# hiimmuc/SpeakerVerification

Hardware: AMD Instinct MI355X
Metric: embeddings/sec (2 s @16 kHz) (higher is better)
Workload: dtype bf16

## Files before the change

speakerverification_amd/csrc/asp_x3.hip:

```cpp
#include "common.h"
#include "kernels.h"

namespace svhip {

namespace {

typedef __attribute__((address_space(3))) void lds_void;
typedef __attribute__((address_space(1))) const void gbl_void;

constexpr int AX_THREADS = 512;
constexpr int AX_PLANE = 32 * 256;
constexpr int AX_RAW = 32 * 512;
constexpr int AX_XSLAB = 32 * 128;
constexpr int AX_NSLOT = 3;
constexpr int AX_XRING = 2 * AX_PLANE + 2 * AX_RAW;
constexpr int AX_LDS = AX_XRING + 8 * AX_NSLOT * AX_XSLAB;
constexpr float AX_L2E = 1.4426950408889634f;

__global__ __launch_bounds__(AX_THREADS, 2) void asp_x3_kernel(AspX3Params p) {
    extern __shared__ __attribute__((aligned(16))) char smem[];
    char* planes = smem;
    char* raw = smem + 2 * AX_PLANE;
    const int ncg = p.C >> 8;
    int b, cg;
    {
        const int id = blockIdx.x, full = (p.B >> 3) * 8 * ncg;
        if (id < full) {
            const int slot = id >> 3;
            b = (slot / ncg) * 8 + (id & 7);
            cg = slot - (slot / ncg) * ncg;
        } else {
            const int q = id - full;
            b = (p.B >> 3) * 8 + q / ncg;
            cg = q - (q / ncg) * ncg;
        }
    }
    const int tid = threadIdx.x, lane = tid & 63;
    const int wave = __builtin_amdgcn_readfirstlane(tid >> 6);
    char* xring = smem + AX_XRING + wave * AX_NSLOT * AX_XSLAB;
    const int r = lane & 31, h = lane >> 5;
    const int cw = cg * 256 + wave * 32;
    const int c = cw + r;
    const int T = p.T;
    const int nt = (T + 31) >> 5;

    bf16x8 wh[8], wl[8];
    {
        const char* wrow = reinterpret_cast<const char*>(p.Ws32) + (int64_t)c * 512;
#pragma unroll
        for (int ks = 0; ks < 8; ++ks) {
            const char* q = wrow + (ks >> 1) * 128 + ((ks & 1) * 16 + 8 * h) * 2;
            wh[ks] = *reinterpret_cast<const bf16x8*>(q);
            wl[ks] = *reinterpret_cast<const bf16x8*>(q + 64);
        }
    }
    const float mref = p.mref[(int64_t)b * p.mref_ld + c];
    const char* abase = reinterpret_cast<const char*>(p.att + (int64_t)b * T * 128) + (lane & 31) * 16;
    const char* xbase = reinterpret_cast<const char*>(p.X + (int64_t)b * T * p.ldx + cw) + (lane & 7) * 16;
    const int64_t xrow = (int64_t)p.ldx * 4;
    auto dma_att = [&](int mt, int buf) {
#pragma unroll
        for (int i = 0; i < 2; ++i) {
            const int f = min(mt * 32 + 4 * wave + 2 * i + (lane >> 5), T - 1);
            __builtin_amdgcn_global_load_lds((gbl_void*)(abase + (int64_t)f * 512), (lds_void*)(raw + buf * AX_RAW + (4 * wave + 2 * i) * 512), 16, 0, CPOL_NT);
        }
    };
    auto dma_x = [&](int mt, int slot) {
#pragma unroll
        for (int i = 0; i < 4; ++i) {
            const int f = min(mt * 32 + 8 * i + (lane >> 3), T - 1);
            __builtin_amdgcn_global_load_lds((gbl_void*)(xbase + f * xrow), (lds_void*)(xring + slot * AX_XSLAB + i * 1024), 16, 0, CPOL_NT);
        }
    };
    const int sfr = tid >> 4;
    const int soff = sfr * 256 + (((tid & 15) ^ (sfr & 15)) << 4);
    auto convert = [&](int buf) {
        const f32x4* q = reinterpret_cast<const f32x4*>(raw + buf * AX_RAW + sfr * 512 + (tid & 15) * 32);
        const f32x4 v0 = q[0], v1 = q[1];
        x3x8_t hi, lo;
#pragma unroll
        for (int j = 0; j < 8; ++j) {
            const float v = j < 4 ? v0[j] : v1[j - 4];
            const x3_t hb = x3_hi(v);
            hi[j] = hb;
            lo[j] = x3_lo(v, hb);
        }
        *reinterpret_cast<x3x8_t*>(planes + soff) = hi;
        *reinterpret_cast<x3x8_t*>(planes + AX_PLANE + soff) = lo;
    };

    auto lds_barrier = [&]() {
        asm volatile("s_waitcnt lgkmcnt(0)" ::: "memory");
        __builtin_amdgcn_s_barrier();
        asm volatile("" ::: "memory");
    };
    float m = -INFINITY, se = 0.0f, s1 = 0.0f, s2 = 0.0f;
    dma_att(0, 0);
    dma_x(0, 0);
    dma_att(1, 1);
    dma_x(1, 1);
    asm volatile("s_waitcnt vmcnt(10)" ::: "memory");
    lds_barrier();
    convert(0);
    lds_barrier();
    int slot = 0;
    for (int mt = 0; mt < nt; ++mt) {
        const int fill = slot == 0 ? 2 : slot - 1;
        dma_att(mt + 2, mt & 1);
        dma_x(mt + 2, fill);
        f32x16 acc;
#pragma unroll
        for (int e = 0; e < 16; ++e) acc[e] = 0.0f;
#pragma unroll
        for (int ks = 0; ks < 8; ++ks) {
            const int o = r * 256 + (((2 * ks + h) ^ (r & 15)) << 4);
            const bf16x8 ah = *reinterpret_cast<const bf16x8*>(planes + o);
            const bf16x8 al = *reinterpret_cast<const bf16x8*>(planes + AX_PLANE + o);
            acc = X3H::mfma32(al, wh[ks], acc);
            acc = X3H::mfma32(ah, wl[ks], acc);
            acc = X3H::mfma32(ah, wh[ks], acc);
        }
        if (mt * 32 + 32 > T) {
#pragma unroll
            for (int e = 0; e < 16; ++e) {
                const int f = mt * 32 + (e & 3) + 8 * (e >> 2) + 4 * h;
                acc[e] = f < T ? acc[e] : -INFINITY;
            }
        }
        float tmax = fmaxf(acc[0], acc[1]);
#pragma unroll
        for (int e = 2; e < 16; e += 2) tmax = fmaxf(fmaxf(acc[e], acc[e + 1]), tmax);
        const float mnew = fmaxf(m, tmax);
        const float mm = mnew == -INFINITY ? 0.0f : mnew;
        const float fs = __builtin_amdgcn_exp2f((m - mm) * AX_L2E);
        se *= fs; s1 *= fs; s2 *= fs;
        const float mb = mm * AX_L2E;
        asm volatile("s_waitcnt vmcnt(12)" ::: "memory");
        const float* xs = reinterpret_cast<const float*>(xring + slot * AX_XSLAB) + r;
#pragma unroll
        for (int e = 0; e < 16; ++e) {
            const float w = __builtin_amdgcn_exp2f(fmaf(acc[e], AX_L2E, -mb));
            const float d = xs[((e & 3) + 8 * (e >> 2) + 4 * h) * 32] - mref;
            const float wd = w * d;
            se += w;
            s1 += wd;
            s2 = fmaf(wd, d, s2);
        }
        m = mnew;
        slot = slot == 2 ? 0 : slot + 1;
        asm volatile("s_waitcnt vmcnt(10)" ::: "memory");
        lds_barrier();
        convert((mt + 1) & 1);
        lds_barrier();
    }
    asm volatile("s_waitcnt vmcnt(0)" ::: "memory");
    const float mo = __shfl_xor(m, 32), seo = __shfl_xor(se, 32), s1o = __shfl_xor(s1, 32), s2o = __shfl_xor(s2, 32);
    const float M = fmaxf(m, mo);
    const float MM = M == -INFINITY ? 0.0f : M;
    const float f1 = __builtin_amdgcn_exp2f((m - MM) * AX_L2E), f2 = __builtin_amdgcn_exp2f((mo - MM) * AX_L2E);
    const float SE = se * f1 + seo * f2, S1 = s1 * f1 + s1o * f2, S2 = s2 * f1 + s2o * f2;
    if (h == 0) {
        const float md = S1 / SE;
        const float mean = mref + md;
        const float sd = sqrtf(fmaxf(S2 / SE - md * md, p.eps));
        const int C = p.C;
        if (p.pooled_raw) {
            p.pooled_raw[(int64_t)b * 2 * C + c] = mean;
            p.pooled_raw[(int64_t)b * 2 * C + C + c] = sd;
        }
        p.pooled_bn[(int64_t)b * 2 * C + c] = fmaf(mean, p.bn_scale[c], p.bn_shift[c]);
        p.pooled_bn[(int64_t)b * 2 * C + C + c] = fmaf(sd, p.bn_scale[C + c], p.bn_shift[C + c]);
    }
}

constexpr int AB_ATT = 32 * 256;
constexpr int AB_XSLAB = 32 * 64;
constexpr int AB_LDS = 2 * AB_ATT + 8 * AX_NSLOT * AB_XSLAB;

__global__ __launch_bounds__(AX_THREADS, 4) void asp_bf16_kernel(AspFusedParams p, const float* __restrict__ mref_all, int mref_ld, int Bn) {
    extern __shared__ __attribute__((aligned(16))) char smem[];
    const int ncg = p.C >> 8;
    int b, cg;
    {
        const int id = blockIdx.x, full = (Bn >> 3) * 8 * ncg;
        if (id < full) {
            const int slot = id >> 3;
            b = (slot / ncg) * 8 + (id & 7);
            cg = slot - (slot / ncg) * ncg;
        } else {
            const int q = id - full;
            b = (Bn >> 3) * 8 + q / ncg;
            cg = q - (q / ncg) * ncg;
        }
    }
    const int tid = threadIdx.x, lane = tid & 63;
    const int wave = __builtin_amdgcn_readfirstlane(tid >> 6);
    char* xring = smem + 2 * AB_ATT + wave * AX_NSLOT * AB_XSLAB;
    const int r = lane & 31, h = lane >> 5;
    const int cw = cg * 256 + wave * 32;
    const int c = cw + r;
    const int T = p.T;
    const int nt = (T + 31) >> 5;

    bf16x8 wf[8];
    {
        const char* wrow = reinterpret_cast<const char*>(p.W) + ((int64_t)c * p.Kp + 8 * h) * 2;
#pragma unroll
        for (int ks = 0; ks < 8; ++ks) wf[ks] = *reinterpret_cast<const bf16x8*>(wrow + ks * 32);
    }
    const float mref = mref_all[(int64_t)b * mref_ld + c];
    const int sfr = tid >> 4;
    const char* abase = reinterpret_cast<const char*>(p.att) + (int64_t)b * T * 256 + (((tid & 15) ^ (sfr & 15)) << 4);
    const char* xbase = reinterpret_cast<const char*>(p.X) + ((int64_t)b * T * p.ldx + cw) * 2 + (lane & 3) * 16;
    const int64_t xrow = (int64_t)p.ldx * 2;
    auto dma_att = [&](int mt, int buf) {
        const int f = min(mt * 32 + sfr, T - 1);
        __builtin_amdgcn_global_load_lds((gbl_void*)(abase + (int64_t)f * 256), (lds_void*)(smem + buf * AB_ATT + wave * 1024), 16, 0, 0);
    };
    auto dma_x = [&](int mt, int slot) {
#pragma unroll
        for (int i = 0; i < 2; ++i) {
            const int f = min(mt * 32 + 16 * i + (lane >> 2), T - 1);
            __builtin_amdgcn_global_load_lds((gbl_void*)(xbase + f * xrow), (lds_void*)(xring + slot * AB_XSLAB + i * 1024), 16, 0, 0);
        }
    };
    auto lds_barrier = [&]() {
        asm volatile("s_waitcnt lgkmcnt(0)" ::: "memory");
        __builtin_amdgcn_s_barrier();
        asm volatile("" ::: "memory");
    };
    float m = -INFINITY, se = 0.0f, s1 = 0.0f, s2 = 0.0f;
    dma_x(0, 0);
    dma_att(0, 0);
    dma_x(1, 1);
    asm volatile("s_waitcnt vmcnt(2)" ::: "memory");
    lds_barrier();
    int slot = 0;
    for (int mt = 0; mt < nt; ++mt) {
        const int buf = mt & 1;
        const int fill = slot == 0 ? 2 : slot - 1;
        dma_att(mt + 1, buf ^ 1);
        dma_x(mt + 2, fill);
        f32x16 acc;
#pragma unroll
        for (int e = 0; e < 16; ++e) acc[e] = 0.0f;
        const char* at = smem + buf * AB_ATT + r * 256;
#pragma unroll
        for (int ks = 0; ks < 8; ++ks) {
            const bf16x8 a = *reinterpret_cast<const bf16x8*>(at + (((2 * ks + h) ^ (r & 15)) << 4));
            acc = __builtin_amdgcn_mfma_f32_32x32x16_bf16(a, wf[ks], acc, 0, 0, 0);
        }
        if (mt * 32 + 32 > T) {
#pragma unroll
            for (int e = 0; e < 16; ++e) {
                const int f = mt * 32 + (e & 3) + 8 * (e >> 2) + 4 * h;
                acc[e] = f < T ? acc[e] : -INFINITY;
            }
        }
        float tmax = fmaxf(acc[0], acc[1]);
#pragma unroll
        for (int e = 2; e < 16; e += 2) tmax = fmaxf(fmaxf(acc[e], acc[e + 1]), tmax);
        const float mnew = fmaxf(m, tmax);
        const float mm = mnew == -INFINITY ? 0.0f : mnew;
        const float fs = __builtin_amdgcn_exp2f((m - mm) * AX_L2E);
        se *= fs; s1 *= fs; s2 *= fs;
        const float mb = mm * AX_L2E;
        const uint16_t* xs = reinterpret_cast<const uint16_t*>(xring + slot * AB_XSLAB) + r;
#pragma unroll
        for (int e = 0; e < 16; ++e) {
            const float w = __builtin_amdgcn_exp2f(fmaf(acc[e], AX_L2E, -mb));
            const float xv = __uint_as_float((uint32_t)xs[((e & 3) + 8 * (e >> 2) + 4 * h) * 32] << 16);
            const float d = xv - mref;
            const float wd = w * d;
            se += w;
            s1 += wd;
            s2 = fmaf(wd, d, s2);
        }
        m = mnew;
        slot = slot == 2 ? 0 : slot + 1;
        asm volatile("s_waitcnt vmcnt(2)" ::: "memory");
        lds_barrier();
    }
    asm volatile("s_waitcnt vmcnt(0)" ::: "memory");
    const float mo = __shfl_xor(m, 32), seo = __shfl_xor(se, 32), s1o = __shfl_xor(s1, 32), s2o = __shfl_xor(s2, 32);
    const float M = fmaxf(m, mo);
    const float MM = M == -INFINITY ? 0.0f : M;
    const float f1 = __builtin_amdgcn_exp2f((m - MM) * AX_L2E), f2 = __builtin_amdgcn_exp2f((mo - MM) * AX_L2E);
    const float SE = se * f1 + seo * f2, S1 = s1 * f1 + s1o * f2, S2 = s2 * f1 + s2o * f2;
    if (h == 0) {
        const float md = S1 / SE;
        const float mean = mref + md;
        const float sd = sqrtf(fmaxf(S2 / SE - md * md, p.eps));
        const int C = p.C;
        if (p.pooled_raw) {
            p.pooled_raw[(int64_t)b * 2 * C + c] = mean;
            p.pooled_raw[(int64_t)b * 2 * C + C + c] = sd;
        }
        p.pooled_bn[(int64_t)b * 2 * C + c] = fmaf(mean, p.bn_scale[c], p.bn_shift[c]);
        p.pooled_bn[(int64_t)b * 2 * C + C + c] = fmaf(sd, p.bn_scale[C + c], p.bn_shift[C + c]);
    }
}

}

hipError_t launch_asp_bf16(const AspFusedParams& p, const float* mref, int mref_ld, int B, hipStream_t stream) {
    if (p.T < 1 || p.C % 256 != 0 || p.Kp != 128 || !p.att || !p.W || !p.X || !mref || !p.pooled_bn || B <= 0 || p.ldx % 8 != 0) return hipErrorInvalidValue;
    static DeviceOnce once;
    hipError_t e = set_max_dynamic_lds(once, reinterpret_cast<const void*>(asp_bf16_kernel), AB_LDS);
    if (e != hipSuccess) return e;
    hipLaunchKernelGGL(asp_bf16_kernel, dim3((p.C / 256) * B), dim3(AX_THREADS), AB_LDS, stream, p, mref, mref_ld, B);
    return hipGetLastError();
}

bool asp_x3_supported(int T, int C, int att_channels, int K) {
    return T >= 1 && C % 256 == 0 && att_channels == 128 && K == 128;
}

hipError_t launch_asp_x3(const AspX3Params& p, int B, hipStream_t stream) {
    if (!asp_x3_supported(p.T, p.C, 128, 128) || !p.att || !p.Ws32 || !p.X || !p.mref || !p.pooled_bn || B <= 0) return hipErrorInvalidValue;
    if (((reinterpret_cast<uintptr_t>(p.att) | reinterpret_cast<uintptr_t>(p.Ws32)) & 15) != 0) return hipErrorInvalidValue;
    static DeviceOnce once;
    hipError_t e = set_max_dynamic_lds(once, reinterpret_cast<const void*>(asp_x3_kernel), AX_LDS);
    if (e != hipSuccess) return e;
    AspX3Params q = p;
    q.B = B;
    hipLaunchKernelGGL(asp_x3_kernel, dim3((p.C / 256) * B), dim3(AX_THREADS), AX_LDS, stream, q);
    return hipGetLastError();
}

}
```

Measured before the change: 57890.

## Software-pipeline ASP bf16 kernel: overlap next tile MFMA with current softmax stats

```diff
diff --git a/speakerverification_amd/csrc/asp_x3.hip b/speakerverification_amd/csrc/asp_x3.hip
--- a/speakerverification_amd/csrc/asp_x3.hip
+++ b/speakerverification_amd/csrc/asp_x3.hip
@@ -7,6 +7,7 @@
 
 typedef __attribute__((address_space(3))) void lds_void;
 typedef __attribute__((address_space(1))) const void gbl_void;
+typedef __attribute__((address_space(3))) const bf16x8 lds_frag;
 
 constexpr int AX_THREADS = 512;
 constexpr int AX_PLANE = 32 * 256;
@@ -176,6 +177,12 @@
 constexpr int AB_ATT = 32 * 256;
 constexpr int AB_XSLAB = 32 * 64;
 constexpr int AB_LDS = 2 * AB_ATT + 8 * AX_NSLOT * AB_XSLAB;
+constexpr int AB_AHEAD = 2;
+#define AB_XREAD(j, e) asm volatile("ds_read_u16_d16_hi %0, %1 offset:%2" : "+v"(xr[j]) : "v"(xa), "n"(((e) & 3) * 64 + ((e) >> 2) * 512) : "memory")
+#define AB_XREREAD(j, e, used) asm volatile("ds_read_u16_d16_hi %0, %1 offset:%2" : "+v"(xr[j]) : "v"(xa), "n"(((e) & 3) * 64 + ((e) >> 2) * 512), "v"(used) : "memory")
+#define AB_XREADS() do { AB_XREAD(0, 0); AB_XREAD(1, 1); AB_XREAD(2, 2); AB_XREAD(3, 3); AB_XREAD(4, 4); AB_XREAD(5, 5); AB_XREAD(6, 6); AB_XREAD(7, 7); } while (0)
+#define AB_XWAIT() do { asm volatile("s_waitcnt lgkmcnt(0)" ::: "memory"); \
+    asm volatile("" : "+v"(xr[0]), "+v"(xr[1]), "+v"(xr[2]), "+v"(xr[3]), "+v"(xr[4]), "+v"(xr[5]), "+v"(xr[6]), "+v"(xr[7]) :: "memory"); } while (0)
 
 __global__ __launch_bounds__(AX_THREADS, 4) void asp_bf16_kernel(AspFusedParams p, const float* __restrict__ mref_all, int mref_ld, int Bn) {
     extern __shared__ __attribute__((aligned(16))) char smem[];
@@ -210,18 +217,18 @@
     }
     const float mref = mref_all[(int64_t)b * mref_ld + c];
     const int sfr = tid >> 4;
-    const char* abase = reinterpret_cast<const char*>(p.att) + (int64_t)b * T * 256 + (((tid & 15) ^ (sfr & 15)) << 4);
-    const char* xbase = reinterpret_cast<const char*>(p.X) + ((int64_t)b * T * p.ldx + cw) * 2 + (lane & 3) * 16;
-    const int64_t xrow = (int64_t)p.ldx * 2;
+    const char* abase = reinterpret_cast<const char*>(p.att) + (int64_t)b * T * 256;
+    const char* xbase = reinterpret_cast<const char*>(p.X) + ((int64_t)b * T * p.ldx + cw) * 2;
+    const uint32_t aoff = ((tid & 15) ^ (sfr & 15)) << 4, xoff = (lane & 3) * 16, xrow = (uint32_t)p.ldx * 2;
     auto dma_att = [&](int mt, int buf) {
         const int f = min(mt * 32 + sfr, T - 1);
-        __builtin_amdgcn_global_load_lds((gbl_void*)(abase + (int64_t)f * 256), (lds_void*)(smem + buf * AB_ATT + wave * 1024), 16, 0, 0);
+        __builtin_amdgcn_global_load_lds((gbl_void*)(abase + (aoff + (uint32_t)f * 256)), (lds_void*)(smem + buf * AB_ATT + wave * 1024), 16, 0, 0);
     };
     auto dma_x = [&](int mt, int slot) {
 #pragma unroll
         for (int i = 0; i < 2; ++i) {
             const int f = min(mt * 32 + 16 * i + (lane >> 2), T - 1);
-            __builtin_amdgcn_global_load_lds((gbl_void*)(xbase + f * xrow), (lds_void*)(xring + slot * AB_XSLAB + i * 1024), 16, 0, 0);
+            __builtin_amdgcn_global_load_lds((gbl_void*)(xbase + (xoff + (uint32_t)f * xrow)), (lds_void*)(xring + slot * AB_XSLAB + i * 1024), 16, 0, 0);
         }
     };
     auto lds_barrier = [&]() {
@@ -230,56 +237,90 @@
         asm volatile("" ::: "memory");
     };
     float m = -INFINITY, se = 0.0f, s1 = 0.0f, s2 = 0.0f;
-    dma_x(0, 0);
-    dma_att(0, 0);
-    dma_x(1, 1);
-    asm volatile("s_waitcnt vmcnt(2)" ::: "memory");
-    lds_barrier();
-    int slot = 0;
-    for (int mt = 0; mt < nt; ++mt) {
-        const int buf = mt & 1;
-        const int fill = slot == 0 ? 2 : slot - 1;
-        dma_att(mt + 1, buf ^ 1);
-        dma_x(mt + 2, fill);
-        f32x16 acc;
-#pragma unroll
-        for (int e = 0; e < 16; ++e) acc[e] = 0.0f;
-        const char* at = smem + buf * AB_ATT + r * 256;
-#pragma unroll
-        for (int ks = 0; ks < 8; ++ks) {
-            const bf16x8 a = *reinterpret_cast<const bf16x8*>(at + (((2 * ks + h) ^ (r & 15)) << 4));
-            acc = __builtin_amdgcn_mfma_f32_32x32x16_bf16(a, wf[ks], acc, 0, 0, 0);
-        }
-        if (mt * 32 + 32 > T) {
-#pragma unroll
-            for (int e = 0; e < 16; ++e) {
-                const int f = mt * 32 + (e & 3) + 8 * (e >> 2) + 4 * h;
-                acc[e] = f < T ? acc[e] : -INFINITY;
+    float xr[8];
+#pragma unroll
+    for (int e = 0; e < 8; ++e) xr[e] = 0.0f;
+    const uint32_t xa0 = (uint32_t)(uintptr_t)(lds_void*)xring + r * 2 + h * 256;
+    int slot = 2;
+    auto pre = [&](int t) {
+        asm volatile("s_waitcnt vmcnt(2)" ::: "memory");
+        lds_barrier();
+        dma_att(t + 2, t & 1);
+        dma_x(t + 2, slot == 0 ? 2 : slot - 1);
+    };
+    auto step = [&](f32x16& as, f32x16& am, const int t, auto SM, auto MM) {
+        constexpr bool sm = decltype(SM)::value, mmf = decltype(MM)::value;
+        const uint32_t at = (uint32_t)(uintptr_t)(lds_void*)smem + ((t + 1) & 1) * AB_ATT + r * 256 + ((h ^ (r & 15)) << 4);
+        auto frag = [&](int ks) { return *(lds_frag*)(uintptr_t)(at ^ (ks << 5)); };
+        bf16x8 af[8];
+        float mnew = m, mb = 0.0f;
+        const uint32_t xa = xa0 + slot * AB_XSLAB;
+        if constexpr (sm) {
+            AB_XREADS();
+            if (t * 32 + 32 > T) {
+#pragma unroll
+                for (int e = 0; e < 16; ++e) {
+                    const int f = t * 32 + (e & 3) + 8 * (e >> 2) + 4 * h;
+                    as[e] = f < T ? as[e] : -INFINITY;
+                }
             }
-        }
-        float tmax = fmaxf(acc[0], acc[1]);
-#pragma unroll
-        for (int e = 2; e < 16; e += 2) tmax = fmaxf(fmaxf(acc[e], acc[e + 1]), tmax);
-        const float mnew = fmaxf(m, tmax);
-        const float mm = mnew == -INFINITY ? 0.0f : mnew;
-        const float fs = __builtin_amdgcn_exp2f((m - mm) * AX_L2E);
-        se *= fs; s1 *= fs; s2 *= fs;
-        const float mb = mm * AX_L2E;
-        const uint16_t* xs = reinterpret_cast<const uint16_t*>(xring + slot * AB_XSLAB) + r;
+            float tmax = fmaxf(as[0], as[1]);
+#pragma unroll
+            for (int e = 2; e < 16; e += 2) tmax = fmaxf(fmaxf(as[e], as[e + 1]), tmax);
+            mnew = fmaxf(m, tmax);
+            const float mm = mnew == -INFINITY ? 0.0f : mnew;
+            const float fs = __builtin_amdgcn_exp2f((m - mm) * AX_L2E);
+            se *= fs; s1 *= fs; s2 *= fs;
+            mb = mm * AX_L2E;
+        }
+        if constexpr (mmf) {
+#pragma unroll
+            for (int e = 0; e < 16; ++e) am[e] = 0.0f;
+#pragma unroll
+            for (int ks = 0; ks < AB_AHEAD; ++ks) af[ks] = frag(ks);
+        }
 #pragma unroll
         for (int e = 0; e < 16; ++e) {
-            const float w = __builtin_amdgcn_exp2f(fmaf(acc[e], AX_L2E, -mb));
-            const float xv = __uint_as_float((uint32_t)xs[((e & 3) + 8 * (e >> 2) + 4 * h) * 32] << 16);
-            const float d = xv - mref;
-            const float wd = w * d;
-            se += w;
-            s1 += wd;
-            s2 = fmaf(wd, d, s2);
+            if ((e & 1) == 0) __builtin_amdgcn_sched_barrier(0);
+            if constexpr (mmf) {
+                if ((e & 1) == 0) {
+                    const int ks = e >> 1;
+                    if (ks + AB_AHEAD < 8) af[ks + AB_AHEAD] = frag(ks + AB_AHEAD);
+                    am = __builtin_amdgcn_mfma_f32_32x32x16_bf16(af[ks], wf[ks], am, 0, 0, 0);
+                }
+            }
+            if constexpr (sm) {
+                if ((e & 7) == 0) AB_XWAIT();
+                const float d = xr[e & 7] - mref;
+                if (e < 8) AB_XREREAD(e, e + 8, d);
+                const float w = __builtin_amdgcn_exp2f(fmaf(as[e], AX_L2E, -mb));
+                const float wd = w * d;
+                se += w;
+                s1 += wd;
+                s2 = fmaf(wd, d, s2);
+            }
         }
         m = mnew;
         slot = slot == 2 ? 0 : slot + 1;
-        asm volatile("s_waitcnt vmcnt(2)" ::: "memory");
-        lds_barrier();
+    };
+    const std::true_type yes;
+    const std::false_type no;
+    f32x16 acc0, acc1;
+    dma_att(0, 0);
+    dma_x(0, 0);
+    pre(-1);
+    step(acc1, acc0, -1, no, yes);
+    int t = 0;
+    for (; t + 1 < nt; t += 2) {
+        pre(t);
+        step(acc0, acc1, t, yes, yes);
+        pre(t + 1);
+        if (t + 2 < nt) step(acc1, acc0, t + 1, yes, yes);
+        else step(acc1, acc0, t + 1, yes, no);
+    }
+    if (t < nt) {
+        pre(t);
+        step(acc0, acc1, t, yes, no);
     }
     asm volatile("s_waitcnt vmcnt(0)" ::: "memory");
     const float mo = __shfl_xor(m, 32), seo = __shfl_xor(se, 32), s1o = __shfl_xor(s1, 32), s2o = __shfl_xor(s2, 32);
@@ -292,6 +333,9 @@
         const float mean = mref + md;
         const float sd = sqrtf(fmaxf(S2 / SE - md * md, p.eps));
         const int C = p.C;
+        int rr = threadIdx.x & 31;
+        asm volatile("" : "+v"(rr));
+        const int c = cw + rr;
         if (p.pooled_raw) {
             p.pooled_raw[(int64_t)b * 2 * C + c] = mean;
             p.pooled_raw[(int64_t)b * 2 * C + C + c] = sd;
@@ -305,6 +349,7 @@
 
 hipError_t launch_asp_bf16(const AspFusedParams& p, const float* mref, int mref_ld, int B, hipStream_t stream) {
     if (p.T < 1 || p.C % 256 != 0 || p.Kp != 128 || !p.att || !p.W || !p.X || !mref || !p.pooled_bn || B <= 0 || p.ldx % 8 != 0) return hipErrorInvalidValue;
+    if ((int64_t)p.T * p.ldx * 2 >= (1ll << 32) || (int64_t)p.T * 256 >= (1ll << 32)) return hipErrorInvalidValue;
     static DeviceOnce once;
     hipError_t e = set_max_dynamic_lds(once, reinterpret_cast<const void*>(asp_bf16_kernel), AB_LDS);
     if (e != hipSuccess) return e;
```

Result: no change. 57950, median of 6 (+0.1%).
